# miczi/OpticalFlowHS

Hardware: AMD Instinct MI355X
Metric: Mpixel*iterations/sec (Horn-Schunck: derivative pass + Jacobi u/v sweeps, frames resident in HBM) (higher is better)
Workload: dtype f32; 1 GPU; a stream of 1920x1080 translating-texture pairs resident in HBM, a new pair every step (two seed pairs alternating), lambda 1, 100 Jacobi iterations, ITER|EPS (eps 1e-6) termination; width=1920, height=1080, iters=100, pairs_per_gpu=1, kernel=strip, fuse_steps=20, threads=1024, rows_per_lane_or_groups=5, tiles_per_launch=243, lds_bytes=131328, hipgraph=True, termination=ITER|EPS (eps 1e-6), loop=stream, call=hsflow_pipeline_submit_device, 6 slots on 2 streams, eps_rerun=0

## Files before the change

opticalflowhs_amd/csrc/hs_kernels_strip.hip.h:

```cpp
#pragma once
#include <type_traits>

#ifndef HS_SWEEP_STAMPS
#define HS_SWEEP_STAMPS 0
#endif
#ifndef HS_DIAG
#define HS_DIAG 0
#endif


namespace hsk {

struct StripGeom {
    int W, H, P;
    long long plane;
    int T, HX;
    int CW, CH;
    int NW;
    int tiles_x, tiles_y;
    int zero_in;
    int org;
    int ey0, ey1;
    const int *pair_list;
};

__device__ __forceinline__ int mirror_index(int i, int n)
{
    if (i < 0) i = -1 - i;
    if (i >= n) i = 2 * n - 1 - i;
    if ((unsigned)i >= (unsigned)n) {
        const int p = 2 * n;
        int m = i % p;
        if (m < 0) m += p;
        i = m < n ? m : p - 1 - m;
    }
    return i;
}

typedef float f2 __attribute__((ext_vector_type(2)));
typedef float f4 __attribute__((ext_vector_type(4)));

struct PersistArgs {
    unsigned *flags;
    unsigned *err;
    float *ub[2], *vb[2];
    int n_phase, T_last;
    unsigned wait_ticks;
};

typedef unsigned u4v __attribute__((ext_vector_type(4)));
__device__ __forceinline__ __amdgpu_buffer_rsrc_t plane_rsrc(float *p)
{
    return __builtin_amdgcn_make_buffer_rsrc((void *)p, 0, 0xFFFFFFFFu, 0x00020000);
}
__device__ __forceinline__ void store_f4_sc1(__amdgpu_buffer_rsrc_t rs, unsigned row_bytes, unsigned lane_bytes, f4 v)
{
    __builtin_amdgcn_raw_buffer_store_b128(__builtin_bit_cast(u4v, v), rs, (int)lane_bytes, (int)row_bytes, 16);
}
__device__ __forceinline__ f4 load_f4_sc1(__amdgpu_buffer_rsrc_t rs, unsigned row_bytes, unsigned lane_bytes)
{
    return __builtin_bit_cast(f4, __builtin_amdgcn_raw_buffer_load_b128(rs, (int)lane_bytes, (int)row_bytes, 16));
}
__device__ __forceinline__ unsigned load_u32_sc1(const unsigned *p)
{
    return __hip_atomic_load(p, __ATOMIC_RELAXED, __HIP_MEMORY_SCOPE_AGENT);
}

__device__ __forceinline__ int hs_lane_now()
{
    unsigned m = ~0u;
    asm volatile("" : "+s"(m));
    return (int)__builtin_amdgcn_mbcnt_hi(m, __builtin_amdgcn_mbcnt_lo(m, 0u));
}

__device__ __forceinline__ f2 f2_fma(f2 a, f2 b, f2 c) { return __builtin_elementwise_fma(a, b, c); }
__device__ __forceinline__ f2 f2_swap(f2 a) { return __builtin_shufflevector(a, a, 1, 0); }
__device__ __forceinline__ f2 sweep_diff(f2 o, f2 n) { return f2_fma(o, f2{4.0f, 4.0f}, -n); }
__device__ __forceinline__ float sweep_diff(float o, float n) { return fmaf(4.0f, o, -n); }

struct RowCoef { f2 alP, alQ, beP, beQ, gaP, gaQ; };

struct Cross { f2 uP, uQ, vP, vQ; };

__device__ __forceinline__ f2 pk_add_swapped(f2 a, f2 b)
{
    f2 r;
    asm("v_pk_add_f32 %0, %1, %2 op_sel:[0,1] op_sel_hi:[1,0]" : "=v"(r) : "v"(a), "v"(b));
    return r;
}

template <int E>
__device__ __forceinline__ void cross_rows(Cross &s, const f2 cuP, const f2 cuQ, const f2 cvP, const f2 cvQ,
                                           const f2 duP, const f2 duQ, const f2 dvP, const f2 dvQ)
{
    if (E == 0) {
        s.uP = duP + cuQ; s.uQ = duQ + cuP;
        s.vP = dvP + cvQ; s.vQ = dvQ + cvP;
    } else {
        s.uQ = pk_add_swapped(duQ, cuQ);
        s.uP.x = duP.x + wave_from_prev_lane(cuP.y); s.uP.y = duP.y + wave_from_next_lane(cuP.x);
        s.vQ = pk_add_swapped(dvQ, cvQ);
        s.vP.x = dvP.x + wave_from_prev_lane(cvP.y); s.vP.y = dvP.y + wave_from_next_lane(cvP.x);
    }
}

template <int E>
__device__ __forceinline__ void strip_row_update(f2 &uP, f2 &uQ, f2 &vP, f2 &vQ, const Cross &sc, const Cross &sp, RowCoef &c)
{
    f2 ubP, ubQ, vbP, vbQ;
    if (E == 0) {
        ubQ = pk_add_swapped(sc.uQ, sp.uQ);
        ubP.x = sc.uP.x + wave_from_prev_lane(sp.uP.y); ubP.y = sc.uP.y + wave_from_next_lane(sp.uP.x);
        vbQ = pk_add_swapped(sc.vQ, sp.vQ);
        vbP.x = sc.vP.x + wave_from_prev_lane(sp.vP.y); vbP.y = sc.vP.y + wave_from_next_lane(sp.vP.x);
    } else {
        ubP = sc.uP + sp.uQ; ubQ = sc.uQ + sp.uP;
        vbP = sc.vP + sp.vQ; vbQ = sc.vQ + sp.vP;
    }
    const f2 qP = f2_fma(c.alP, ubP, f2_fma(c.beP, vbP, c.gaP));
    const f2 qQ = f2_fma(c.alQ, ubQ, f2_fma(c.beQ, vbQ, c.gaQ));
    uP = f2_fma(-c.alP, qP, ubP);
    vP = f2_fma(-c.beP, qP, vbP);
    uQ = f2_fma(-c.alQ, qQ, ubQ);
    vQ = f2_fma(-c.beQ, qQ, vbQ);
    c.gaP *= 4.0f;
    c.gaQ *= 4.0f;
}

struct FrameSrc {
    int PA, PB;
    uint8_t *keepA, *keepB;
};

template <int R, bool EXT = false>
__device__ __forceinline__ void strip_derive(const uint8_t *__restrict__ fA, const uint8_t *__restrict__ fB,
                                             const StripGeom &g, long long base, int x0, int y0, int dir, bool xin,
                                             uint4 (&lc)[R], const FrameSrc fs = FrameSrc{0, 0, nullptr, nullptr},
                                             const unsigned keep = 0)
{
    const int PA = EXT ? fs.PA : g.P, PB = EXT ? fs.PB : g.P;
    const int mode = xin ? 0 : ((x0 < 0 || (g.W & 3) == 0) ? 1 : 2);
    int xg = x0, xb[4] = {0, 0, 0, 0};
    unsigned flipx = 0;
    if (mode == 1) {
        xg = x0 < 0 ? -x0 - 4 : 2 * g.W - x0 - 4;
        if (xg < 0 || xg + 4 > g.W) xg = 0;
        flipx = 0xFu;
    } else if (mode == 2) {
#pragma unroll
        for (int k = 0; k < 4; k++) {
            xb[k] = mirror_index(x0 + k, g.W);
            if (x0 + k >= g.W) flipx |= 1u << k;
        }
    }
    uint32_t wa[R + 2], wbv[R];
#pragma unroll
    for (int j = 0; j < R + 2; j++)
        wa[j] = *(const uint32_t *)(fA + base + (long long)mirror_index(y0 + dir * (j - 1), g.H) * PA + (mode == 2 ? 0 : xg));
#pragma unroll
    for (int r = 0; r < R; r++)
        wbv[r] = *(const uint32_t *)(fB + base + (long long)mirror_index(y0 + dir * r, g.H) * PB + (mode == 2 ? 0 : xg));
    if (mode == 1) {
#pragma unroll
        for (int j = 0; j < R + 2; j++) wa[j] = __builtin_bswap32(wa[j]);
#pragma unroll
        for (int r = 0; r < R; r++) wbv[r] = __builtin_bswap32(wbv[r]);
    }
    if (__builtin_amdgcn_ballot_w64(mode == 2) != 0) {
        if (mode == 2) {
            auto bytes = [&](const uint8_t *row) -> uint32_t {
                return (uint32_t)row[xb[0]] | ((uint32_t)row[xb[1]] << 8) | ((uint32_t)row[xb[2]] << 16) | ((uint32_t)row[xb[3]] << 24);
            };
#pragma unroll
            for (int j = 0; j < R + 2; j++) wa[j] = bytes(fA + base + (long long)mirror_index(y0 + dir * (j - 1), g.H) * PA);
#pragma unroll
            for (int r = 0; r < R; r++) wbv[r] = bytes(fB + base + (long long)mirror_index(y0 + dir * r, g.H) * PB);
        }
    }
    if constexpr (EXT) {
        if (fs.keepA != nullptr) {
#pragma unroll
            for (int r = 0; r < R; r++) {
                if ((keep >> r) & 1u) {
                    const long long o = base + (long long)(y0 + dir * r) * g.P + x0;
                    *(uint32_t *)(fs.keepA + o) = wa[r + 1];
                    *(uint32_t *)(fs.keepB + o) = wbv[r];
                }
            }
        }
    }
    int a[R + 2][6];
#pragma unroll
    for (int j = 0; j < R + 2; j++) {
        const uint32_t wd = wa[j];
        a[j][0] = (int)((uint32_t)__builtin_amdgcn_update_dpp(0, (int)wd, 0x138, 0xF, 0xF, true) >> 24);
        a[j][5] = (int)((uint32_t)__builtin_amdgcn_update_dpp(0, (int)wd, 0x130, 0xF, 0xF, true) & 0xFFu);
#pragma unroll
        for (int k = 0; k < 4; k++) a[j][k + 1] = (int)((wd >> (8 * k)) & 0xFFu);
    }
#pragma unroll
    for (int r = 0; r < R; r++) {
        const int y = y0 + dir * r;
        const uint32_t wb = wbv[r];
        const bool yflip = (y < 0 || y >= g.H) != (dir < 0);
        uint32_t o[4];
#pragma unroll
        for (int k = 0; k < 4; k++) {
            int ix8 = (a[r][k + 2] + 2 * a[r + 1][k + 2] + a[r + 2][k + 2]) - (a[r][k] + 2 * a[r + 1][k] + a[r + 2][k]);
            int iy8 = (a[r + 2][k] + 2 * a[r + 2][k + 1] + a[r + 2][k + 2]) - (a[r][k] + 2 * a[r][k + 1] + a[r][k + 2]);
            if ((flipx >> k) & 1u) ix8 = -ix8;
            if (yflip) iy8 = -iy8;
            o[k] = pack_deriv(ix8, iy8, (int)((wb >> (8 * k)) & 0xFFu) - a[r + 1][k + 1]);
        }
        lc[r] = make_uint4(o[0], o[1], o[2], o[3]);
    }
}


struct TileId { int tile, slot, pair, bx, by; };
template <bool LISTED, bool SCALAR>
__device__ __forceinline__ TileId tile_decode(const StripGeom &g)
{
    const int tpp = g.tiles_x * g.tiles_y;
    const int tile = xcd_contiguous_tile(blockIdx.x, gridDim.x);
    const int slot = tile / tpp;
    const int t2 = tile - slot * tpp;
    int pair = slot;
    if constexpr (LISTED) {
        if (g.pair_list) pair = g.pair_list[slot];
    }
    if constexpr (SCALAR) pair = __builtin_amdgcn_readfirstlane(pair);
    const int by = t2 / g.tiles_x, bx = t2 - by * g.tiles_x;
    return TileId{tile, slot, pair, bx, by};
}

#define HS_ROW_IN_CORE(j, y, T, CH, H) ((j) >= (T) && (j) < (T) + (CH) && (y) >= 0 && (y) < (H))
__device__ __forceinline__ bool row_in_core(const int j, const int y, const int T, const int CH, const int H)
{
    return HS_ROW_IN_CORE(j, y, T, CH, H);
}
__device__ __forceinline__ int row_dist(const int j, const int T, const int CH)
{
    return j < T ? T - j : (j >= T + CH ? j - (T + CH - 1) : 0);
}
__device__ __forceinline__ bool lane_in_core(const int x0, const int xl, const StripGeom &g)
{
    return (x0 >= 0) && (x0 < g.W) && (xl >= g.HX) && (xl < g.HX + g.CW);
}

__device__ __forceinline__ bool group_inside(const int x0, const int W) { return (x0 >= 0) && (x0 + 3 < W); }
struct ColRule { int xg, rev, slow; };
__device__ __forceinline__ ColRule column_rule(const int x0, const int W, const bool side, const bool inside)
{
    ColRule c{x0, 0, 0};
    if (side && !inside) {
        if (x0 < 0 && -x0 <= W) { c.xg = -x0 - 4; c.rev = 1; }
        else if (x0 >= W && (W & 3) == 0 && 2 * W - x0 - 4 >= 0) { c.xg = 2 * W - x0 - 4; c.rev = 1; }
        else { c.xg = 0; c.slow = 1; }
    }
    return c;
}

__device__ __forceinline__ void unpack(const float4 u, const float4 v, const uint4 cw, const float ilambda,
                                       f2 &uP, f2 &uQ, f2 &vP, f2 &vQ, RowCoef &c)
{
    constexpr int iPx = 0, iPy = 3, iQx = 1, iQy = 2;
    const float lu4[4] = {u.x, u.y, u.z, u.w}, lv4[4] = {v.x, v.y, v.z, v.w};
    uP = f2{lu4[iPx], lu4[iPy]}; uQ = f2{lu4[iQx], lu4[iQy]};
    vP = f2{lv4[iPx], lv4[iPy]}; vQ = f2{lv4[iQx], lv4[iQy]};
    float al[4], be[4], ga[4];
    const uint32_t cc[4] = {cw.x, cw.y, cw.z, cw.w};
#pragma unroll
    for (int p = 0; p < 4; p++) sweep_coefs(cc[p], ilambda, al[p], be[p], ga[p]);
    c.alP = f2{al[iPx], al[iPy]}; c.alQ = f2{al[iQx], al[iQy]};
    c.beP = f2{be[iPx], be[iPy]}; c.beQ = f2{be[iQx], be[iQy]};
    c.gaP = f2{ga[iPx], ga[iPy]} * 4.0f; c.gaQ = f2{ga[iQx], ga[iQy]} * 4.0f;
}

template <int R, bool DERIV, class RowOf>
__device__ __forceinline__ void load_rows(const uint32_t *coef, const float *u_in, const float *v_in, const StripGeom &g,
                                          const long long base, const int xg, const RowOf image_row,
                                          float4 (&lu)[R], float4 (&lv)[R], uint4 (&lc)[R])
{
#pragma unroll
    for (int r = 0; r < R; r++) {
        const long long off = base + (long long)mirror_index(image_row(r), g.H) * g.P + xg;
        const long long off_uv = g.zero_in ? (long long)xg : off;
        lc[r] = make_uint4(0u, 0u, 0u, 0u);
        if constexpr (!DERIV) {
            lu[r] = *(const float4 *)(u_in + off_uv);
            lv[r] = *(const float4 *)(v_in + off_uv);
            lc[r] = *(const uint4 *)(coef + off);
        } else {
            lu[r] = lv[r] = make_float4(0.f, 0.f, 0.f, 0.f);
        }
    }
    if constexpr (DERIV) {
        if (!g.zero_in) {
#pragma unroll
            for (int r = 0; r < R; r++) {
                const long long off = base + (long long)mirror_index(image_row(r), g.H) * g.P + xg;
                lu[r] = *(const float4 *)(u_in + off);
                lv[r] = *(const float4 *)(v_in + off);
            }
        }
    }
}

template <int R, bool DERIV, class RowOf>
__device__ __forceinline__ void load_rows_slow(const uint32_t *coef, const float *u_in, const float *v_in, const StripGeom &g,
                                               const float ilambda, const long long base, const int x0, const bool slow,
                                               const RowOf image_row, float4 (&lu)[R], float4 (&lv)[R], uint4 (&lc)[R],
                                               f2 (&uP)[R], f2 (&uQ)[R], f2 (&vP)[R], f2 (&vQ)[R], RowCoef (&cf)[R])
{
    if (__builtin_amdgcn_ballot_w64(slow) != 0) {
        if (slow) {
            const int xa = mirror_index(x0, g.W), xb = mirror_index(x0 + 1, g.W),
                      xc = mirror_index(x0 + 2, g.W), xd = mirror_index(x0 + 3, g.W);
#pragma unroll
            for (int r = 0; r < R; r++) {
                const long long row = base + (long long)mirror_index(image_row(r), g.H) * g.P;
                {
                    const float *uv = u_in + (g.zero_in ? 0 : row), *vv = v_in + (g.zero_in ? 0 : row);
                    lu[r] = make_float4(uv[xa], uv[xb], uv[xc], uv[xd]);
                    lv[r] = make_float4(vv[xa], vv[xb], vv[xc], vv[xd]);
                }
                if constexpr (!DERIV) {
                    const uint32_t *cv = coef + row;
                    lc[r] = make_uint4(cv[xa], cv[xb], cv[xc], cv[xd]);
                    unpack(lu[r], lv[r], lc[r], ilambda, uP[r], uQ[r], vP[r], vQ[r], cf[r]);
                }
            }
        }
    }
}

#define HS_MIRROR_ROW(DERIV, rev, lu, lv, uP, uQ, vP, vQ, cf)                                      \
    do {                                                                                           \
        if constexpr (DERIV) {                                                                     \
            if (rev) {                                                                             \
                lu = make_float4(lu.w, lu.z, lu.y, lu.x);                                          \
                lv = make_float4(lv.w, lv.z, lv.y, lv.x);                                          \
            }                                                                                      \
        } else {                                                                                   \
            uP = rev ? f2_swap(uP) : uP; uQ = rev ? f2_swap(uQ) : uQ;                              \
            vP = rev ? f2_swap(vP) : vP; vQ = rev ? f2_swap(vQ) : vQ;                              \
            cf.alP = rev ? f2_swap(cf.alP) : cf.alP; cf.alQ = rev ? f2_swap(cf.alQ) : cf.alQ;      \
            cf.beP = rev ? f2_swap(cf.beP) : cf.beP; cf.beQ = rev ? f2_swap(cf.beQ) : cf.beQ;      \
            cf.gaP = rev ? f2_swap(cf.gaP) : cf.gaP; cf.gaQ = rev ? f2_swap(cf.gaQ) : cf.gaQ;      \
        }                                                                                          \
    } while (0)

#define HS_LOAD_PHASE(R, DERIV, side, inside, x0, base, image_row, lu, lv, lc, uP, uQ, vP, vQ, cf)                     \
    do {                                                                                                               \
        const ColRule col_ = column_rule(x0, g.W, side, inside);                                                       \
        const bool mirrored_ = col_.rev != 0;                                                                          \
        load_rows<R, DERIV>(coef, u_in, v_in, g, base, col_.xg, image_row, lu, lv, lc);                                \
        if constexpr (!DERIV) {                                                                                        \
            _Pragma("unroll") for (int r = 0; r < R; r++)                                                              \
                unpack(lu[r], lv[r], lc[r], ilambda, uP[r], uQ[r], vP[r], vQ[r], cf[r]);                               \
        }                                                                                                              \
        if (side) {                                                                                                    \
            _Pragma("unroll") for (int r = 0; r < R; r++)                                                              \
                HS_MIRROR_ROW(DERIV, mirrored_, lu[r], lv[r], uP[r], uQ[r], vP[r], vQ[r], cf[r]);                      \
            load_rows_slow<R, DERIV>(coef, u_in, v_in, g, ilambda, base, x0, col_.slow != 0, image_row, lu, lv, lc,    \
                                     uP, uQ, vP, vQ, cf);                                                              \
        }                                                                                                              \
    } while (0)

template <int R, class RowOf>
__device__ __forceinline__ void store_deriv_rows(uint32_t *coef_w, const StripGeom &g, const long long base,
                                                 const int x0, const unsigned rowcore, const RowOf image_row, const uint4 (&lc)[R])
{
#pragma unroll
    for (int r = 0; r < R; r++)
        if ((rowcore >> r) & 1u) *(uint4 *)(coef_w + base + (long long)image_row(r) * g.P + x0) = lc[r];
}

template <int R, class RowOf>
__device__ __forceinline__ void store_flow_rows(float *u_out, float *v_out, const StripGeom &g,
                                                const long long base, const int x0, const unsigned rowcore, const RowOf image_row,
                                                const f2 (&uP)[R], const f2 (&uQ)[R], const f2 (&vP)[R], const f2 (&vQ)[R])
{
#pragma unroll
    for (int r = 0; r < R; r++) {
        if ((rowcore >> r) & 1u) {
            const long long off = base + (long long)image_row(r) * g.P + x0;
            const float fin = __builtin_ldexpf(1.0f, -2 * g.T);
            *(float4 *)(u_out + off) = make_float4(uP[r].x * fin, uQ[r].x * fin, uQ[r].y * fin, uP[r].y * fin);
            *(float4 *)(v_out + off) = make_float4(vP[r].x * fin, vQ[r].x * fin, vQ[r].y * fin, vP[r].y * fin);
        }
    }
}

__device__ __forceinline__ unsigned long long store_stamps(unsigned long long *stamps, const unsigned long long st0,
                                                           const unsigned long long sr0, const unsigned long long st1,
                                                           const unsigned long long st2, const int tile)
{
    __builtin_amdgcn_s_waitcnt(0);
    unsigned long long *o = stamps + (size_t)blockIdx.x * 8;
    o[0] = st0; o[1] = st1; o[2] = st2;
    const unsigned long long st3 = __builtin_amdgcn_s_memtime();
    o[3] = st3;
    o[4] = sr0; o[5] = __builtin_amdgcn_s_memrealtime();
    o[6] = (unsigned long long)__builtin_amdgcn_s_getreg(((4 - 1) << 11) | (0 << 6) | 20);
    o[7] = (unsigned long long)tile;
    return st3;
}

template <class Lane>
__device__ __forceinline__ void eps_put_max(const float *vals, const int NW, const Lane lane_id, unsigned *word)
{
    float x = lane_id() < NW ? vals[lane_id()] : 0.f;
    x = wave_max_nonneg(x);
    if (lane_id() == 0) *word = __float_as_uint(x);
}
#define HS_EPS_FOLD_SWEEP(EPS, e, s, w, NW, lane, eps_lds, eps_out, eps_stride)                                        \
    do {                                                                                                               \
        const float unscale_ = __builtin_ldexpf(1.0f, -2 * ((s) + 1));                                                 \
        if (EPS == 3) {                                                                                                \
            const float e_ = wave_max_nonneg(e) * unscale_;                                                            \
            if ((lane) == 0) eps_lds[16 + (w)] = e_;                                                                   \
        }                                                                                                              \
        if (EPS == 1) {                                                                                                \
            const float e_ = wave_max_nonneg(e) * unscale_;                                                            \
            if ((lane) == 0) eps_lds[((s) & 1) * 16 + (w)] = e_;                                                       \
            if ((s) > 0 && (w) == 0) {                                                                                 \
                float x_ = (lane) < (NW) ? eps_lds[(((s) - 1) & 1) * 16 + (lane)] : 0.f;                               \
                x_ = wave_max_nonneg(x_);                                                                              \
                if ((lane) == 0) eps_out[(size_t)((s) - 1) * (eps_stride) + blockIdx.x] = __float_as_uint(x_);         \
            }                                                                                                          \
        }                                                                                                              \
    } while (0)
template <int EPS, bool COUNTS, class Lane>
__device__ __forceinline__ void eps_tail(const int T, const int seen_n, const bool wit_sum, const int w, const int NW, const Lane lane_id,
                                         float *eps_lds, unsigned *eps_out, unsigned *wit_out, const int eps_stride)
{
    if (EPS == 1) {
        __syncthreads();
        if (w == 0) eps_put_max(eps_lds + ((T - 1) & 1) * 16, NW, lane_id, eps_out + (size_t)(T - 1) * eps_stride + blockIdx.x);
    }
    if (EPS == 2 || EPS == 3) {
        const int witnessed = EPS == 3 ? T - 1 : T;
        if (lane_id() == 0) eps_lds[w] = COUNTS ? (float)seen_n : (seen_n == witnessed ? __builtin_inff() : 0.f);
        __syncthreads();
        if (w == 0) {
            const float x = lane_id() < NW ? eps_lds[lane_id()] : 0.f;
            const float n = wit_sum ? wave_sum16(x) : wave_max_nonneg(x);
            if (lane_id() == 0) wit_out[blockIdx.x] = __float_as_uint(!COUNTS ? n : n == (float)witnessed ? __builtin_inff() : 0.f);
            if (EPS == 3) eps_put_max(eps_lds + 16, NW, lane_id, eps_out + (size_t)eps_stride + blockIdx.x);
        }
    }
}

constexpr int kSweepLast = 16;
template <int EPS, bool TWO, bool MARK_LAST = false, class Sweep>
__device__ __forceinline__ void run_sweeps(const int &T, const Sweep &sweep)
{
    constexpr int kLast = MARK_LAST ? kSweepLast : 0;
    if constexpr (EPS == 3) {
#pragma unroll 1
        for (int s = 0; s + 1 < T; s++) sweep(s, std::integral_constant<int, 2>{});
        sweep(T - 1, std::integral_constant<int, 1 + kLast>{});
    } else if constexpr (EPS != 1) {
        int s = 0;
        if constexpr (TWO) {
#pragma unroll 1
            for (; s + 2 < T; s += 2) {
                sweep(s, std::integral_constant<int, EPS>{});
                sweep(s + 1, std::integral_constant<int, EPS>{});
            }
        }
#pragma unroll 1
        for (; s + 1 < T; s++) sweep(s, std::integral_constant<int, EPS>{});
        sweep(T - 1, std::integral_constant<int, EPS + kLast>{});
    } else {
        const int n = T;
#pragma unroll 1
        for (int s = 0; s < n; s++) sweep(s, std::integral_constant<int, EPS>{});
    }
}

template <int R, int NTMAX, int EPS, int E0, bool DERIV, bool PERSIST = false>
__device__ __forceinline__ void strip_body(const uint32_t *__restrict__ coef,
                                                        const float *__restrict__ u_in,
                                                        const float *__restrict__ v_in,
                                                        float *__restrict__ u_out,
                                                        float *__restrict__ v_out, const StripGeom g,
                                                        const float ilambda,
                                                        unsigned *__restrict__ eps_out, const int eps_stride,
                                                        unsigned long long *__restrict__ stamps,
                                                        const float eps_thr, const uint8_t *__restrict__ fA,
                                                        const uint8_t *__restrict__ fB, uint32_t *__restrict__ coef_w,
                                                        const FrameSrc fs, const PersistArgs pa = PersistArgs())
{
    static_assert(!PERSIST || EPS == 0 || EPS == 2, "the persistent form runs plain or witness phases");
    extern __shared__ __attribute__((aligned(16))) float4 ex[];
    unsigned long long st0 = 0, sr0 = 0, st1 = 0, st2 = 0;
    if (stamps) { st0 = __builtin_amdgcn_s_memtime(); sr0 = __builtin_amdgcn_s_memrealtime(); }
    const int lane = threadIdx.x & 63;
    const int w = __builtin_amdgcn_readfirstlane(threadIdx.x >> 6);
    const int NW = g.NW;
    float *eps_lds = (float *)(ex + (size_t)2 * NW * 4 * 64);
    const TileId tl = tile_decode<!PERSIST, false>(g);
    const int x0 = tl.bx * g.CW - g.HX + 4 * lane;
    const int y0 = tl.by * g.CH - g.T + w * R;
    const long long base = (long long)tl.pair * g.plane;
    const bool xin = group_inside(x0, g.W);
    const bool rev = (R & 1) != 0 && ((y0 + g.org) & 1) != 0;
    auto img_row = [&](int r) { return rev ? R - 1 - r : r; };
    auto image_row = [&](int r) { return y0 + img_row(r); };

    f2 uP[R], uQ[R], vP[R], vQ[R];
    RowCoef cf[R];
    float4 lu[R], lv[R];
    uint4 lc[R];
    const int rx0 = tl.bx * g.CW - g.HX;
    const bool xedge = !(rx0 >= 0 && rx0 + 256 <= g.W);
    HS_LOAD_PHASE(R, DERIV, xedge, xin, x0, base, image_row, lu, lv, lc, uP, uQ, vP, vQ, cf);
    unsigned rowcore = 0;
    int rdist[R];
#pragma unroll
    for (int r = 0; r < R; r++) {
        const int j = w * R + img_row(r);
        const int y = image_row(r);
        if constexpr (DERIV) {
            if (row_in_core(j, y, g.T, g.CH, g.H)) rowcore |= 1u << r;
        } else {
            if (HS_ROW_IN_CORE(j, y, g.T, g.CH, g.H)) rowcore |= 1u << r;
        }
        rdist[r] = row_dist(j, g.T, g.CH);
    }
    const bool lanecore = lane_in_core(x0, 4 * lane, g);
    if constexpr (DERIV) {
        const unsigned keep = (fs.keepA != nullptr && lanecore) ? rowcore : 0u;
        strip_derive<R, true>(fA, fB, g, base, x0, rev ? y0 + R - 1 : y0, rev ? -1 : 1, xin, lc, fs, keep);
#pragma unroll
        for (int r = 0; r < R; r++) unpack(lu[r], lv[r], lc[r], ilambda, uP[r], uQ[r], vP[r], vQ[r], cf[r]);
    }
    const int pr = g.W - 1 - x0;
    constexpr bool LANE_HW = EPS != 0 || PERSIST;
    const auto lane_id = [&]() __attribute__((always_inline)) { return LANE_HW ? hs_lane_now() : lane; };
    unsigned epscore = 0;
    if (EPS != 0) {
#pragma unroll
        for (int r = 0; r < R; r++) {
            const int y = image_row(r);
            if (((rowcore >> r) & 1u) && y >= g.ey0 && y < g.ey1) epscore |= 1u << r;
        }
    }
    if (DERIV && lanecore) store_deriv_rows<R>(coef_w, g, base, x0, rowcore, image_row, lc);

#define HS_LIKELY(c) (PERSIST ? !!(c) : __builtin_expect(!!(c), 1))
#define HS_ACT(r) HS_LIKELY(((act >> (r)) & 1u) != 0u)
#define HS_ROW(r, PE, SC, SP)                                                                      \
    do {                                                                                           \
        if (HS_LIKELY(((actr >> (r)) & 1u) != 0u)) {                                               \
            f2 ouP, ouQ, ovP, ovQ;                                                                 \
            if (EM == 1) { ouP = uP[r]; ouQ = uQ[r]; ovP = vP[r]; ovQ = vQ[r]; }                   \
            if (HS_DIAG & 8) uP[r] += SC.uP + SP.uP;                                               \
            else strip_row_update<PE>(uP[r], uQ[r], vP[r], vQ[r], SC, SP, cf[r]);                  \
            if (EM == 1) {                                                                         \
                if ((epscore >> (r)) & 1u) {  \
                    const f2 dUP = sweep_diff(ouP, uP[r]), dUQ = sweep_diff(ouQ, uQ[r]), dVP = sweep_diff(ovP, vP[r]), dVQ = sweep_diff(ovQ, vQ[r]); \
                    if (HS_LIKELY(!xedge)) {  \
                        e = fmaxf(fmaxf(e, fabsf(dUP.x)), fabsf(dUP.y));                           \
                        e = fmaxf(fmaxf(e, fabsf(dUQ.x)), fabsf(dUQ.y));                           \
                        e = fmaxf(fmaxf(e, fabsf(dVP.x)), fabsf(dVP.y));                           \
                        e = fmaxf(fmaxf(e, fabsf(dVQ.x)), fabsf(dVQ.y));                           \
                    } else {                                                                       \
                         \
                        e = fmaxf(e, fmaxf(fabsf(dUP.x), fabsf(dVP.x)));                           \
                        if (pr >= 1) e = fmaxf(e, fmaxf(fabsf(dUQ.x), fabsf(dVQ.x)));              \
                        if (pr >= 2) e = fmaxf(e, fmaxf(fabsf(dUQ.y), fabsf(dVQ.y)));              \
                        if (pr >= 3) e = fmaxf(e, fmaxf(fabsf(dUP.y), fabsf(dVP.y)));              \
                    }                                                                              \
                }                                                                                  \
            }                                                                                      \
        }                                                                                          \
    } while (0)
#define HS_CROSS(S, PE, A, B)                                                                      \
    do {                                                                                           \
        if (HS_LIKELY(((actb >> (A)) & 1u) != 0u)) {                               \
            if (HS_DIAG & 8) S.uP = uP[A] + uP[B];                                                 \
            else cross_rows<PE>(S, uP[A], uQ[A], vP[A], vQ[A], uP[B], uQ[B], vP[B], vQ[B]);        \
        }                                                                                          \
    } while (0)
#define HS_PUBLISH(buf, ln)                                                                         \
    do {                                                                                           \
        float4 *exw = ex + ((size_t)((buf) * NW + w) * 4) * 64 + (ln);                             \
        exw[0] = make_float4(uP[0].x, uP[0].y, uQ[0].x, uQ[0].y);                                  \
        exw[64] = make_float4(vP[0].x, vP[0].y, vQ[0].x, vQ[0].y);                                 \
        exw[128] = make_float4(uP[R - 1].x, uP[R - 1].y, uQ[R - 1].x, uQ[R - 1].y);                \
        exw[192] = make_float4(vP[R - 1].x, vP[R - 1].y, vQ[R - 1].x, vQ[R - 1].y);                \
    } while (0)

    if (stamps) st1 = __builtin_amdgcn_s_memtime();
    const bool nrev = (R & 1) != 0 && !rev;
    const int wa = w > 0 ? w - 1 : w, sa = w > 0 ? (nrev ? 0 : 2) : 0;
    const int wb = w < NW - 1 ? w + 1 : w, sb = w < NW - 1 ? (nrev ? 2 : 0) : 2;
    const int wu = rev ? wb : wa, su = rev ? sb : sa;
    const int wd = rev ? wa : wb, sd = rev ? sa : sb;
    int seen_n = 0;
    const unsigned long long wit_mask = (epscore & 1u) ? __builtin_amdgcn_ballot_w64(lanecore) : 0ull;
    const int core_here = min(g.CH, g.H - tl.by * g.CH);
    const int wit_lo = (g.T + R - 1) / R, wit_n = (g.T + core_here) / R - wit_lo;
    const bool wit_rot = wit_n > 0;
    const int wit_per = wit_rot ? wit_n : 1;
    const int wit_cnt0 = !wit_rot ? 0 : (w >= wit_lo && w < wit_lo + wit_n) ? w - wit_lo : (1 << 30);
    int wit_cnt = wit_cnt0;
    int Tp = g.T;
    unsigned long long act_lo = 0, act_hi = 0;
    auto sweep = [&](const int s, auto em_tag) __attribute__((always_inline)) {
        constexpr int EM = decltype(em_tag)::value & (kSweepLast - 1);
        constexpr bool IN_LOOP = (decltype(em_tag)::value & kSweepLast) == 0;
#if HS_DIAG & 4
        unsigned act = ~0u;
#else
        unsigned act = (unsigned)((act_lo << s) >> 32) & (unsigned)(act_hi >> (24 + s));
#endif
        unsigned actb = act | (act >> 1), actr = act;
        if constexpr (EPS != 1) asm volatile("" : "+s"(act), "+s"(actb), "+s"(actr));
        const float thr_s = __int_as_float(__float_as_int(eps_thr) + ((s + 1) << 24));
#if HS_DIAG & 1
        const float4 hu4 = make_float4(uP[0].x, uP[0].y, uQ[0].x, uQ[0].y), hv4 = make_float4(vP[0].x, vP[0].y, vQ[0].x, vQ[0].y);
        const float4 du4 = make_float4(uP[R - 1].x, uP[R - 1].y, uQ[R - 1].x, uQ[R - 1].y), dv4 = make_float4(vP[R - 1].x, vP[R - 1].y, vQ[R - 1].x, vQ[R - 1].y);
#else
        const int lane_l = lane_id();
        const float4 *eu = ex + ((size_t)((s & 1) * NW + wu) * 4 + su) * 64 + lane_l;
        const float4 *ed = ex + ((size_t)((s & 1) * NW + wd) * 4 + sd) * 64 + lane_l;
        const float4 hu4 = eu[0], hv4 = eu[64];
        const float4 du4 = ed[0], dv4 = ed[64];
#endif
        const f2 huP = f2{hu4.x, hu4.y}, huQ = f2{hu4.z, hu4.w}, hvP = f2{hv4.x, hv4.y}, hvQ = f2{hv4.z, hv4.w};
        const f2 duP = f2{du4.x, du4.y}, duQ = f2{du4.z, du4.w}, dvP = f2{dv4.x, dv4.y}, dvQ = f2{dv4.z, dv4.w};

        float e = 0.f;
        constexpr int EL = E0 ^ ((R - 1) & 1);
        Cross sA, s0, sK, sL;
        const bool wturn = EM == 2 && (PERSIST ? wit_cnt == 0 : __builtin_expect(wit_cnt == 0, 0));
        float w0 = 0.f;
        if (wturn) w0 = uP[0].x;
        if (HS_ACT(0)) cross_rows<E0 ^ 1>(sA, huP, huQ, hvP, hvQ, uP[0], uQ[0], vP[0], vQ[0]);
        if (R == 1) {
            if (HS_ACT(0)) cross_rows<E0>(s0, uP[0], uQ[0], vP[0], vQ[0], duP, duQ, dvP, dvQ);
        } else {
            constexpr int R1 = R > 1 ? 1 : 0;
            HS_CROSS(s0, E0, 0, R1);
        }
        HS_ROW(0, E0, s0, sA);
        if (EM == 2) {
            if (wturn) seen_n += (__builtin_amdgcn_ballot_w64(fabsf(sweep_diff(w0, uP[0].x)) >= thr_s) & wit_mask) != 0 ? 1 : 0;
            wit_cnt = wturn ? wit_per - 1 : wit_cnt - 1;
        }
        if (R >= 2) {
            constexpr int RM = R > 2 ? R - 2 : 0;
            if (HS_ACT(R - 1)) cross_rows<EL>(sL, uP[R - 1], uQ[R - 1], vP[R - 1], vQ[R - 1], duP, duQ, dvP, dvQ);
                if (R >= 3) HS_CROSS(sK, EL ^ 1, RM, R - 1);
            if (R == 2) HS_ROW(R - 1, EL, sL, s0);
            else HS_ROW(R - 1, EL, sL, sK);
        }
#if !(HS_DIAG & 1)
        if (s + 1 < Tp) HS_PUBLISH((s + 1) & 1, lane_l);
#endif
        if (R >= 3) {
            Cross sp = s0;
            Cross scs[R], sc1;
#pragma unroll
            for (int r = 1; r < R - 1; r++) {
                Cross &sc = IN_LOOP && EM != 1 ? scs[r] : sc1;
                if (r == R - 2) sc = sK;
                else {
                    const int rn = r + 1 < R ? r + 1 : r;
                    if (r & 1) HS_CROSS(sc, E0 ^ 1, r, rn);
                    else HS_CROSS(sc, E0, r, rn);
                }
                if (r & 1) HS_ROW(r, E0 ^ 1, sc, sp);
                else HS_ROW(r, E0, sc, sp);
                sp = sc;
            }
        }
        if constexpr (EM == 1) HS_EPS_FOLD_SWEEP(EPS, lanecore ? e : 0.f, s, w, NW, lane_id(), eps_lds, eps_out, eps_stride);
#if !(HS_DIAG & 2)
        if (s + 1 < Tp) __syncthreads();
#endif
#if HS_SWEEP_STAMPS
        if (stamps && gridDim.x <= 8192 && threadIdx.x == 0)
            stamps[(size_t)gridDim.x * 8 + (size_t)blockIdx.x * 32 + (s & 31)] = __builtin_amdgcn_s_memtime();
#endif
    };
    if (rowcore == (1u << R) - 1u) __builtin_amdgcn_s_setprio(1);
    int ph = 0;
    unsigned flag_base = 0;
    unsigned long long pt_sweep = 0, pt_pub = 0, pt_wait = 0, pt_load = 0, pt0 = 0, pt_first = 0;
    if constexpr (PERSIST) {
        if (w == 0) flag_base = (unsigned)__builtin_amdgcn_readfirstlane((int)load_u32_sc1(pa.flags + tl.tile));
    }
#pragma unroll 1
    for (;;) {
    if constexpr (PERSIST) {
        Tp = ph == pa.n_phase - 1 ? pa.T_last : g.T;
        seen_n = 0;
        wit_cnt = wit_cnt0;
        if (stamps && ph == 0) pt_first = pt0 = __builtin_amdgcn_s_memtime();
    }
    {
        static_assert(R <= 8, "the trapezoid tables hold 8 rows per lane");
        const int n0 = min(max(g.T - Tp + 1 - w * R, -32), R), m0 = min(max(w * R + R + 1 - g.T - g.CH - Tp, -32), R);
        act_lo = ~0ull << (32 + (rev ? m0 : n0));
        act_hi = ~0ull >> (40 - R + (rev ? n0 : m0));
    }
    HS_PUBLISH(0, lane_id());
    __syncthreads();
    if (PERSIST && stamps && ph > 0) {
        const unsigned long long t = __builtin_amdgcn_s_memtime();
        pt_load += t - pt0;
        pt0 = t;
    }
    run_sweeps<EPS, false, true>(Tp, sweep);
    unsigned *const eps_ph = PERSIST ? eps_out + (size_t)ph * eps_stride : eps_out;
    eps_tail<EPS, true>(Tp, seen_n, wit_rot, w, NW, lane_id, eps_lds, eps_out, eps_ph, eps_stride);
    if (stamps) st2 = __builtin_amdgcn_s_memtime();

    if constexpr (!PERSIST) {
        int lane_s = lane_id();
        if constexpr (!LANE_HW) asm volatile("" : "+v"(lane_s));
        const int x0s = tl.bx * g.CW - g.HX + 4 * lane_s;
        if (lanecore) store_flow_rows<R>(u_out, v_out, g, base, x0s, rowcore, image_row, uP, uQ, vP, vQ);
        break;
    } else {
        if (stamps) { pt_sweep += st2 - pt0; pt0 = st2; }
        const __amdgpu_buffer_rsrc_t pu = plane_rsrc(pa.ub[ph & 1]), pv = plane_rsrc(pa.vb[ph & 1]);
        const float fin = __builtin_ldexpf(1.0f, -2 * Tp);
        const int lane_x = lane_id();
        const int x0x = tl.bx * g.CW - g.HX + 4 * lane_x;
        const ColRule colx = column_rule(x0x, g.W, xedge, group_inside(x0x, g.W));
        const int xgx = colx.xg;
        const bool xrevx = colx.rev != 0;
#pragma unroll
        for (int r = 0; r < R; r++) {
            if ((rowcore >> r) & 1u) {
                uP[r] *= fin; uQ[r] *= fin; vP[r] *= fin; vQ[r] *= fin;
                if (lanecore) {
                    const unsigned row = 4u * (unsigned)(base + (long long)image_row(r) * g.P);
                    store_f4_sc1(pu, row, 4u * (unsigned)x0x, f4{uP[r].x, uQ[r].x, uQ[r].y, uP[r].y});
                    store_f4_sc1(pv, row, 4u * (unsigned)x0x, f4{vP[r].x, vQ[r].x, vQ[r].y, vP[r].y});
                }
            }
        }
        if (ph == pa.n_phase - 1) break;
#pragma unroll
        for (int r = 0; r < R; r++) {
            const int nact = Tp - rdist[r] > 0 ? Tp - rdist[r] : 0;
            const float back = __builtin_ldexpf(1.0f, -2 * nact);
            cf[r].gaP *= back; cf[r].gaQ *= back;
        }
        asm volatile("s_waitcnt vmcnt(0)" ::: "memory");
        __syncthreads();
        if (stamps) { const unsigned long long t = __builtin_amdgcn_s_memtime(); pt_pub += t - pt0; pt0 = t; }
        int *const dead_lds = (int *)(eps_lds + 31);
        if (w == 0) {
            const unsigned target = flag_base + (unsigned)ph + 1u;
            if (lane_id() == 0) __hip_atomic_store(pa.flags + tl.tile, target, __ATOMIC_RELAXED, __HIP_MEMORY_SCOPE_AGENT);
            int nb = -1;
            if (lane_id() < 8) {
                const int k = lane_id() < 4 ? lane_id() : lane_id() + 1;
                const int nx = tl.bx + k % 3 - 1, ny = tl.by + k / 3 - 1;
                if (nx >= 0 && nx < g.tiles_x && ny >= 0 && ny < g.tiles_y) nb = tl.slot * g.tiles_x * g.tiles_y + ny * g.tiles_x + nx;
            } else if (lane_id() == 8) nb = (int)gridDim.x;
            const unsigned long long t0 = __builtin_amdgcn_s_memrealtime();
            int dead = 0;
            for (;;) {
                unsigned v = target;
                if (nb >= 0) v = load_u32_sc1(pa.flags + nb);
                const bool aborted = lane_id() == 8 && v != 0u;
                const bool behind = lane_id() < 8 && (int)(v - target) < 0;
                if (__builtin_amdgcn_ballot_w64(aborted) != 0) { dead = 1; break; }
                if (__builtin_amdgcn_ballot_w64(behind) == 0) break;
                if (__builtin_amdgcn_s_memrealtime() - t0 > (unsigned long long)pa.wait_ticks) {
                    dead = 1;
                    if (lane_id() == 0) {
                        __hip_atomic_store(pa.flags + gridDim.x, 1u, __ATOMIC_RELAXED, __HIP_MEMORY_SCOPE_AGENT);
                        __hip_atomic_store(pa.err, 1u, __ATOMIC_RELAXED, __HIP_MEMORY_SCOPE_SYSTEM);
                    }
                    break;
                }
                __builtin_amdgcn_s_sleep(4);
            }
            if (lane_id() == 0) *dead_lds = dead;
        }
        __syncthreads();
        if (__builtin_amdgcn_readfirstlane(*dead_lds)) return;
        if (stamps) { const unsigned long long t = __builtin_amdgcn_s_memtime(); pt_wait += t - pt0; pt0 = t; }
        {
            f4 tu[R], tv[R];
#pragma unroll
            for (int r = 0; r < R; r++) {
                const unsigned row = 4u * (unsigned)(base + (long long)mirror_index(image_row(r), g.H) * g.P);
                tu[r] = f4{uP[r].x, uQ[r].x, uQ[r].y, uP[r].y};
                tv[r] = f4{vP[r].x, vQ[r].x, vQ[r].y, vP[r].y};
                if (!((rowcore >> r) & 1u) || !lanecore) {
                    tu[r] = load_f4_sc1(pu, row, 4u * (unsigned)xgx);
                    tv[r] = load_f4_sc1(pv, row, 4u * (unsigned)xgx);
                }
            }
#pragma unroll
            for (int r = 0; r < R; r++) {
                if (xrevx) {
                    tu[r] = f4{tu[r].w, tu[r].z, tu[r].y, tu[r].x};
                    tv[r] = f4{tv[r].w, tv[r].z, tv[r].y, tv[r].x};
                }
                uP[r] = f2{tu[r].x, tu[r].w}; uQ[r] = f2{tu[r].y, tu[r].z};
                vP[r] = f2{tv[r].x, tv[r].w}; vQ[r] = f2{tv[r].y, tv[r].z};
            }
        }
        ph++;
    }
    }
#undef HS_ROW
#undef HS_ACT
#undef HS_LIKELY
#undef HS_CROSS
#undef HS_PUBLISH
    if (stamps && threadIdx.x == 0) {
        const unsigned long long st3 = store_stamps(stamps, st0, sr0, st1, st2, tl.tile);
        if (PERSIST && gridDim.x <= 8192) {
            unsigned long long *q = stamps + (size_t)gridDim.x * 8 + (size_t)blockIdx.x * 32;
            q[0] = pt_sweep; q[1] = pt_pub; q[2] = pt_wait; q[3] = pt_load; q[4] = pt_first - st1; q[5] = st3 - st2;
        }
    }
}

template <int R, int NTMAX, int EPS, int E0>
__global__ __launch_bounds__(NTMAX) void k_jacobi_strip(const uint32_t *__restrict__ coef,
                                                        const float *__restrict__ u_in,
                                                        const float *__restrict__ v_in,
                                                        float *__restrict__ u_out,
                                                        float *__restrict__ v_out, const StripGeom g,
                                                        const float ilambda,
                                                        unsigned *__restrict__ eps_out, const int eps_stride,
                                                        unsigned long long *__restrict__ stamps,
                                                        const float eps_thr)
{
    strip_body<R, NTMAX, EPS, E0, false>(coef, u_in, v_in, u_out, v_out, g, ilambda, eps_out, eps_stride, stamps, eps_thr,
                                     nullptr, nullptr, nullptr, FrameSrc{0, 0, nullptr, nullptr});
}

template <int R, int NTMAX, int EPS, int E0>
__global__ __launch_bounds__(NTMAX) void k_jacobi_strip_deriv(const uint8_t *__restrict__ fA,
                                                              const uint8_t *__restrict__ fB, const FrameSrc fs,
                                                              uint32_t *__restrict__ coef_w,
                                                              const float *__restrict__ u_in,
                                                              const float *__restrict__ v_in,
                                                              float *__restrict__ u_out,
                                                              float *__restrict__ v_out, const StripGeom g,
                                                              const float ilambda,
                                                              unsigned *__restrict__ eps_out, const int eps_stride,
                                                              unsigned long long *__restrict__ stamps,
                                                              const float eps_thr)
{
    strip_body<R, NTMAX, EPS, E0, true>(nullptr, u_in, v_in, u_out, v_out, g, ilambda, eps_out, eps_stride, stamps, eps_thr,
                                    fA, fB, coef_w, fs);
}

template <int R, int NTMAX, int EPS, int E0, bool DERIV>
__global__ __launch_bounds__(NTMAX) void k_jacobi_strip_persist(const uint8_t *__restrict__ fA,
                                                                const uint8_t *__restrict__ fB,
                                                                uint32_t *coef_rw,
                                                                const float *__restrict__ u_in,
                                                                const float *__restrict__ v_in, const StripGeom g,
                                                                const float ilambda,
                                                                unsigned *__restrict__ eps_out, const int eps_stride,
                                                                unsigned long long *__restrict__ stamps,
                                                                const float eps_thr, const PersistArgs pa)
{
    strip_body<R, NTMAX, EPS, E0, DERIV, true>(coef_rw, u_in, v_in, nullptr, nullptr, g, ilambda, eps_out, eps_stride, stamps, eps_thr,
                                               fA, fB, coef_rw, FrameSrc{g.P, g.P, nullptr, nullptr}, pa);
}

__device__ __forceinline__ float lane_xor32(float x, bool lower)
{
    const unsigned b = __float_as_uint(x);
    const auto r = __builtin_amdgcn_permlane32_swap(b, b, false, false);
    return __uint_as_float(lower ? r[0] : r[1]);
}

template <int R, int NTMAX, int EPS, int E0, bool DERIV>
__device__ __forceinline__ void fold_body(const uint32_t *__restrict__ coef,
                                                       const float *__restrict__ u_in,
                                                       const float *__restrict__ v_in,
                                                       float *__restrict__ u_out,
                                                       float *__restrict__ v_out, const StripGeom g,
                                                       const float ilambda,
                                                       unsigned *__restrict__ eps_out, const int eps_stride,
                                                       unsigned long long *__restrict__ stamps,
                                                       const float eps_thr, const uint8_t *__restrict__ fA,
                                                       const uint8_t *__restrict__ fB, uint32_t *__restrict__ coef_w)
{
    extern __shared__ __attribute__((aligned(16))) float4 ex[];
    unsigned long long st0 = 0, sr0 = 0, st1 = 0, st2 = 0;
    if (stamps) { st0 = __builtin_amdgcn_s_memtime(); sr0 = __builtin_amdgcn_s_memrealtime(); }
    const int lane = threadIdx.x & 63, hl = lane & 31;
    const bool lower = lane >= 32;
    const int w = __builtin_amdgcn_readfirstlane(threadIdx.x >> 6);
    const int NW = g.NW;
    float *eps_lds = (float *)(ex + (size_t)2 * NW * 2 * 2 * 32);
    const TileId tl = tile_decode<true, true>(g);
    const int rx0 = tl.bx * g.CW - g.HX;
    const int x0 = rx0 + 4 * hl;
    const int yb = tl.by * g.CH - g.T + w * 2 * R;
    const long long base = (long long)tl.pair * g.plane;
    const bool xin = group_inside(x0, g.W);
    auto blk_row = [&](int r) { return lower ? 2 * R - 1 - r : r; };
    auto image_row = [&](int r) { return yb + blk_row(r); };
    const auto lane_id = [&]() { return lane; };

    f2 uP[R], uQ[R], vP[R], vQ[R];
    RowCoef cf[R];
    float4 lu[R], lv[R];
    uint4 lc[R];
    const bool side = !(rx0 >= 0 && rx0 + 128 <= g.W);
    HS_LOAD_PHASE(R, DERIV, side, xin, x0, base, image_row, lu, lv, lc, uP, uQ, vP, vQ, cf);
    if constexpr (DERIV) {
        strip_derive<R>(fA, fB, g, base, x0, lower ? yb + 2 * R - 1 : yb, lower ? -1 : 1, xin, lc);
#pragma unroll
        for (int r = 0; r < R; r++) unpack(lu[r], lv[r], lc[r], ilambda, uP[r], uQ[r], vP[r], vQ[r], cf[r]);
    }
    unsigned rowcore = 0;
    int rdist[R];
#pragma unroll
    for (int r = 0; r < R; r++) {
        const int jl = w * 2 * R + blk_row(r), y = image_row(r);
        if (HS_ROW_IN_CORE(jl, y, g.T, g.CH, g.H)) rowcore |= 1u << r;
        const int du = row_dist(w * 2 * R + r, g.T, g.CH), dd = row_dist(w * 2 * R + 2 * R - 1 - r, g.T, g.CH);
        rdist[r] = du < dd ? du : dd;
    }
    const bool lanecore = lane_in_core(x0, 4 * hl, g);
    const int pr = g.W - 1 - x0;
    if (DERIV && lanecore) store_deriv_rows<R>(coef_w, g, base, x0, rowcore, image_row, lc);

#define HF_ROW(r, PE, SC, SP)                                                                      \
    do {                                                                                           \
        if (rdist[r] <= last) {                                                                    \
            f2 ouP, ouQ, ovP, ovQ;                                                                 \
            if (EM == 1) { ouP = uP[r]; ouQ = uQ[r]; ovP = vP[r]; ovQ = vQ[r]; }                   \
            strip_row_update<PE>(uP[r], uQ[r], vP[r], vQ[r], SC, SP, cf[r]);                       \
            if (EM == 1) {                                                                         \
                if (((rowcore >> (r)) & 1u) && lanecore) {                                         \
                       \
                    e = fmaxf(e, fmaxf(fabsf(sweep_diff(ouP.x, uP[r].x)), fabsf(sweep_diff(ovP.x, vP[r].x))));           \
                    if (pr >= 1) e = fmaxf(e, fmaxf(fabsf(sweep_diff(ouQ.x, uQ[r].x)), fabsf(sweep_diff(ovQ.x, vQ[r].x)))); \
                    if (pr >= 2) e = fmaxf(e, fmaxf(fabsf(sweep_diff(ouQ.y, uQ[r].y)), fabsf(sweep_diff(ovQ.y, vQ[r].y)))); \
                    if (pr >= 3) e = fmaxf(e, fmaxf(fabsf(sweep_diff(ouP.y, uP[r].y)), fabsf(sweep_diff(ovP.y, vP[r].y)))); \
                }                                                                                  \
            }                                                                                      \
        }                                                                                          \
        __builtin_amdgcn_sched_barrier(0);                                                         \
    } while (0)
#define HF_CROSS(S, PE, A, B)                                                                      \
    do {                                                                                           \
        if (rdist[A] <= last || rdist[B] <= last)                                                  \
            cross_rows<PE>(S, uP[A], uQ[A], vP[A], vQ[A], uP[B], uQ[B], vP[B], vQ[B]);             \
    } while (0)
#define HF_SLOT(buf, ww, hh) (ex + ((size_t)(((buf) * NW + (ww)) * 2 + (hh)) * 2) * 32)
#define HF_PUBLISH(buf)                                                                            \
    do {                                                                                           \
        float4 *exw = HF_SLOT(buf, w, lower ? 1 : 0) + hl;                                         \
        exw[0] = make_float4(uP[0].x, uP[0].y, uQ[0].x, uQ[0].y);                                  \
        exw[32] = make_float4(vP[0].x, vP[0].y, vQ[0].x, vQ[0].y);                                 \
    } while (0)

    HF_PUBLISH(0);
    __syncthreads();
    if (stamps) st1 = __builtin_amdgcn_s_memtime();
    const int wo = lower ? (w < NW - 1 ? w + 1 : w) : (w > 0 ? w - 1 : w);
    const int ho = lower ? (w < NW - 1 ? 0 : 1) : (w > 0 ? 1 : 0);
    int seen_n = 0;
    const unsigned long long wit_mask = __builtin_amdgcn_ballot_w64((rowcore & 1u) && lanecore);
    auto sweep = [&](const int s, auto em_tag) __attribute__((always_inline)) {
        constexpr int EM = decltype(em_tag)::value;
        const int last = g.T - 1 - s;
        const float thr_s = __int_as_float(__float_as_int(eps_thr) + ((s + 1) << 24));
        const float4 *eo = HF_SLOT(s & 1, wo, ho) + hl;
        const float4 h4u = eo[0], h4v = eo[32];
        const f2 ouP_ = f2{h4u.x, h4u.y}, ouQ_ = f2{h4u.z, h4u.w}, ovP_ = f2{h4v.x, h4v.y}, ovQ_ = f2{h4v.z, h4v.w};
        const f2 iuP = f2{lane_xor32(uP[R - 1].x, lower), lane_xor32(uP[R - 1].y, lower)};
        const f2 iuQ = f2{lane_xor32(uQ[R - 1].x, lower), lane_xor32(uQ[R - 1].y, lower)};
        const f2 ivP = f2{lane_xor32(vP[R - 1].x, lower), lane_xor32(vP[R - 1].y, lower)};
        const f2 ivQ = f2{lane_xor32(vQ[R - 1].x, lower), lane_xor32(vQ[R - 1].y, lower)};
        float e = 0.f;
        const float w0 = uP[0].x;
        Cross sp, sc;
        if (rdist[0] <= last) cross_rows<E0 ^ 1>(sp, ouP_, ouQ_, ovP_, ovQ_, uP[0], uQ[0], vP[0], vQ[0]);
#pragma unroll
        for (int r = 0; r < R; r++) {
            const int rn = r + 1 < R ? r + 1 : r;
            if (r == R - 1) {
                if (rdist[r] <= last) {
                    if (r & 1) cross_rows<E0 ^ 1>(sc, uP[r], uQ[r], vP[r], vQ[r], iuP, iuQ, ivP, ivQ);
                    else cross_rows<E0>(sc, uP[r], uQ[r], vP[r], vQ[r], iuP, iuQ, ivP, ivQ);
                }
            } else if (r & 1) HF_CROSS(sc, E0 ^ 1, r, rn);
            else HF_CROSS(sc, E0, r, rn);
            if (r & 1) HF_ROW(r, E0 ^ 1, sc, sp);
            else HF_ROW(r, E0, sc, sp);
            if (r == 0) {
                if (EM == 2)
                    seen_n += (__builtin_amdgcn_ballot_w64(fabsf(sweep_diff(w0, uP[0].x)) >= thr_s) & wit_mask) != 0 ? 1 : 0;
                if (s + 1 < g.T) HF_PUBLISH((s + 1) & 1);
            }
            sp = sc;
        }
        if constexpr (EM == 1) HS_EPS_FOLD_SWEEP(EPS, e, s, w, NW, lane, eps_lds, eps_out, eps_stride);
        if (s + 1 < g.T) __syncthreads();
    };
    run_sweeps<EPS, true>(g.T, sweep);
    eps_tail<EPS, false>(g.T, seen_n, false, w, NW, lane_id, eps_lds, eps_out, eps_out, eps_stride);
#undef HF_ROW
#undef HF_CROSS
#undef HF_PUBLISH
#undef HF_SLOT
    if (stamps) st2 = __builtin_amdgcn_s_memtime();

    if (lanecore) store_flow_rows<R>(u_out, v_out, g, base, x0, rowcore, image_row, uP, uQ, vP, vQ);
    if (stamps && threadIdx.x == 0) store_stamps(stamps, st0, sr0, st1, st2, tl.tile);
}

template <int R, int NTMAX, int EPS, int E0>
__global__ __launch_bounds__(NTMAX) void k_jacobi_fold(const uint32_t *__restrict__ coef,
                                                       const float *__restrict__ u_in,
                                                       const float *__restrict__ v_in,
                                                       float *__restrict__ u_out,
                                                       float *__restrict__ v_out, const StripGeom g,
                                                       const float ilambda,
                                                       unsigned *__restrict__ eps_out, const int eps_stride,
                                                       unsigned long long *__restrict__ stamps,
                                                       const float eps_thr)
{
    fold_body<R, NTMAX, EPS, E0, false>(coef, u_in, v_in, u_out, v_out, g, ilambda, eps_out, eps_stride, stamps, eps_thr,
                                    nullptr, nullptr, nullptr);
}

template <int R, int NTMAX, int EPS, int E0>
__global__ __launch_bounds__(NTMAX) void k_jacobi_fold_deriv(const uint8_t *__restrict__ fA,
                                                             const uint8_t *__restrict__ fB,
                                                             uint32_t *__restrict__ coef_w,
                                                             const float *__restrict__ u_in,
                                                             const float *__restrict__ v_in,
                                                             float *__restrict__ u_out,
                                                             float *__restrict__ v_out, const StripGeom g,
                                                             const float ilambda,
                                                             unsigned *__restrict__ eps_out, const int eps_stride,
                                                             unsigned long long *__restrict__ stamps,
                                                             const float eps_thr)
{
    fold_body<R, NTMAX, EPS, E0, true>(nullptr, u_in, v_in, u_out, v_out, g, ilambda, eps_out, eps_stride, stamps, eps_thr,
                                   fA, fB, coef_w);
}

#undef HS_ROW_IN_CORE
#undef HS_EPS_FOLD_SWEEP
#undef HS_LOAD_PHASE
#undef HS_MIRROR_ROW

}
```

Baseline: 1.802 million Mpix*iter/s.

## Add unguarded full-strip sweep variant with scheduling barriers for interior waves

```diff
diff --git a/opticalflowhs_amd/csrc/hs_kernels_strip.hip.h b/opticalflowhs_amd/csrc/hs_kernels_strip.hip.h
--- a/opticalflowhs_amd/csrc/hs_kernels_strip.hip.h
+++ b/opticalflowhs_amd/csrc/hs_kernels_strip.hip.h
@@ -454,30 +454,31 @@
 }
 
 constexpr int kSweepLast = 16;
-template <int EPS, bool TWO, bool MARK_LAST = false, class Sweep>
+constexpr int kSweepFull = 32;
+template <int EPS, bool TWO, bool MARK_LAST = false, int MORE = 0, class Sweep>
 __device__ __forceinline__ void run_sweeps(const int &T, const Sweep &sweep)
 {
     constexpr int kLast = MARK_LAST ? kSweepLast : 0;
     if constexpr (EPS == 3) {
 #pragma unroll 1
-        for (int s = 0; s + 1 < T; s++) sweep(s, std::integral_constant<int, 2>{});
+        for (int s = 0; s + 1 < T; s++) sweep(s, std::integral_constant<int, 2 + MORE>{});
         sweep(T - 1, std::integral_constant<int, 1 + kLast>{});
     } else if constexpr (EPS != 1) {
         int s = 0;
         if constexpr (TWO) {
 #pragma unroll 1
             for (; s + 2 < T; s += 2) {
-                sweep(s, std::integral_constant<int, EPS>{});
-                sweep(s + 1, std::integral_constant<int, EPS>{});
+                sweep(s, std::integral_constant<int, EPS + MORE>{});
+                sweep(s + 1, std::integral_constant<int, EPS + MORE>{});
             }
         }
 #pragma unroll 1
-        for (; s + 1 < T; s++) sweep(s, std::integral_constant<int, EPS>{});
+        for (; s + 1 < T; s++) sweep(s, std::integral_constant<int, EPS + MORE>{});
         sweep(T - 1, std::integral_constant<int, EPS + kLast>{});
     } else {
         const int n = T;
 #pragma unroll 1
-        for (int s = 0; s < n; s++) sweep(s, std::integral_constant<int, EPS>{});
+        for (int s = 0; s < n; s++) sweep(s, std::integral_constant<int, EPS + MORE>{});
     }
 }
 
@@ -552,10 +553,15 @@
     if (DERIV && lanecore) store_deriv_rows<R>(coef_w, g, base, x0, rowcore, image_row, lc);
 
 #define HS_LIKELY(c) (PERSIST ? !!(c) : __builtin_expect(!!(c), 1))
-#define HS_ACT(r) HS_LIKELY(((act >> (r)) & 1u) != 0u)
+#define HS_GUARD(c) (FULL || HS_LIKELY(c))
+#define HS_FENCE()                                                                                 \
+    do {                                                                                           \
+        if constexpr (FULL) __builtin_amdgcn_sched_barrier(0);                                     \
+    } while (0)
+#define HS_ACT(r) HS_GUARD(((act >> (r)) & 1u) != 0u)
 #define HS_ROW(r, PE, SC, SP)                                                                      \
     do {                                                                                           \
-        if (HS_LIKELY(((actr >> (r)) & 1u) != 0u)) {                                               \
+        if (HS_GUARD(((actr >> (r)) & 1u) != 0u)) {                                                \
             f2 ouP, ouQ, ovP, ovQ;                                                                 \
             if (EM == 1) { ouP = uP[r]; ouQ = uQ[r]; ovP = vP[r]; ovQ = vQ[r]; }                   \
             if (HS_DIAG & 8) uP[r] += SC.uP + SP.uP;                                               \
@@ -578,13 +584,15 @@
                 }                                                                                  \
             }                                                                                      \
         }                                                                                          \
+        HS_FENCE();                                                                                \
     } while (0)
 #define HS_CROSS(S, PE, A, B)                                                                      \
     do {                                                                                           \
-        if (HS_LIKELY(((actb >> (A)) & 1u) != 0u)) {                               \
+        if (HS_GUARD(((actb >> (A)) & 1u) != 0u)) {                                \
             if (HS_DIAG & 8) S.uP = uP[A] + uP[B];                                                 \
             else cross_rows<PE>(S, uP[A], uQ[A], vP[A], vQ[A], uP[B], uQ[B], vP[B], vQ[B]);        \
         }                                                                                          \
+        if constexpr (!DERIV) HS_FENCE();                                                          \
     } while (0)
 #define HS_PUBLISH(buf, ln)                                                                         \
     do {                                                                                           \
@@ -614,19 +622,19 @@
     auto sweep = [&](const int s, auto em_tag) __attribute__((always_inline)) {
         constexpr int EM = decltype(em_tag)::value & (kSweepLast - 1);
         constexpr bool IN_LOOP = (decltype(em_tag)::value & kSweepLast) == 0;
-#if HS_DIAG & 4
+        constexpr bool FULL = (decltype(em_tag)::value & kSweepFull) != 0;
         unsigned act = ~0u;
-#else
-        unsigned act = (unsigned)((act_lo << s) >> 32) & (unsigned)(act_hi >> (24 + s));
+#if !(HS_DIAG & 4)
+        if constexpr (!FULL) act = (unsigned)((act_lo << s) >> 32) & (unsigned)(act_hi >> (24 + s));
 #endif
         unsigned actb = act | (act >> 1), actr = act;
-        if constexpr (EPS != 1) asm volatile("" : "+s"(act), "+s"(actb), "+s"(actr));
+        if constexpr (EPS != 1 && !FULL) asm volatile("" : "+s"(act), "+s"(actb), "+s"(actr));
         const float thr_s = __int_as_float(__float_as_int(eps_thr) + ((s + 1) << 24));
 #if HS_DIAG & 1
         const float4 hu4 = make_float4(uP[0].x, uP[0].y, uQ[0].x, uQ[0].y), hv4 = make_float4(vP[0].x, vP[0].y, vQ[0].x, vQ[0].y);
         const float4 du4 = make_float4(uP[R - 1].x, uP[R - 1].y, uQ[R - 1].x, uQ[R - 1].y), dv4 = make_float4(vP[R - 1].x, vP[R - 1].y, vQ[R - 1].x, vQ[R - 1].y);
 #else
-        const int lane_l = lane_id();
+        const int lane_l = FULL ? hs_lane_now() : lane_id();
         const float4 *eu = ex + ((size_t)((s & 1) * NW + wu) * 4 + su) * 64 + lane_l;
         const float4 *ed = ex + ((size_t)((s & 1) * NW + wd) * 4 + sd) * 64 + lane_l;
         const float4 hu4 = eu[0], hv4 = eu[64];
@@ -640,8 +648,12 @@
         Cross sA, s0, sK, sL;
         const bool wturn = EM == 2 && (PERSIST ? wit_cnt == 0 : __builtin_expect(wit_cnt == 0, 0));
         float w0 = 0.f;
-        if (wturn) w0 = uP[0].x;
+        if (wturn) {
+            w0 = uP[0].x;
+            if constexpr (FULL) asm volatile("" : "+v"(w0));
+        }
         if (HS_ACT(0)) cross_rows<E0 ^ 1>(sA, huP, huQ, hvP, hvQ, uP[0], uQ[0], vP[0], vQ[0]);
+        if constexpr (!DERIV) HS_FENCE();
         if (R == 1) {
             if (HS_ACT(0)) cross_rows<E0>(s0, uP[0], uQ[0], vP[0], vQ[0], duP, duQ, dvP, dvQ);
         } else {
@@ -656,6 +668,7 @@
         if (R >= 2) {
             constexpr int RM = R > 2 ? R - 2 : 0;
             if (HS_ACT(R - 1)) cross_rows<EL>(sL, uP[R - 1], uQ[R - 1], vP[R - 1], vQ[R - 1], duP, duQ, dvP, dvQ);
+            if constexpr (!DERIV) HS_FENCE();
                 if (R >= 3) HS_CROSS(sK, EL ^ 1, RM, R - 1);
             if (R == 2) HS_ROW(R - 1, EL, sL, s0);
             else HS_ROW(R - 1, EL, sL, sK);
@@ -663,6 +676,7 @@
 #if !(HS_DIAG & 1)
         if (s + 1 < Tp) HS_PUBLISH((s + 1) & 1, lane_l);
 #endif
+        HS_FENCE();
         if (R >= 3) {
             Cross sp = s0;
             Cross scs[R], sc1;
@@ -689,7 +703,8 @@
             stamps[(size_t)gridDim.x * 8 + (size_t)blockIdx.x * 32 + (s & 31)] = __builtin_amdgcn_s_memtime();
 #endif
     };
-    if (rowcore == (1u << R) - 1u) __builtin_amdgcn_s_setprio(1);
+    const bool full_strip = rowcore == (1u << R) - 1u;
+    if (full_strip) __builtin_amdgcn_s_setprio(1);
     int ph = 0;
     unsigned flag_base = 0;
     unsigned long long pt_sweep = 0, pt_pub = 0, pt_wait = 0, pt_load = 0, pt0 = 0, pt_first = 0;
@@ -717,7 +732,14 @@
         pt_load += t - pt0;
         pt0 = t;
     }
-    run_sweeps<EPS, false, true>(Tp, sweep);
+    if constexpr (!PERSIST && (EPS == 0 || EPS == 2) && R >= 4) {
+        unsigned take_full = (unsigned)__builtin_amdgcn_readfirstlane(full_strip ? 1 : 0), take_guarded;
+        asm volatile("" : "+s"(take_full));
+        if (take_full != 0u) run_sweeps<EPS, false, true, kSweepFull>(Tp, sweep);
+        take_guarded = take_full ^ 1u;
+        asm volatile("" : "+s"(take_guarded));
+        if (take_guarded != 0u) run_sweeps<EPS, false, true>(Tp, sweep);
+    } else run_sweeps<EPS, false, true>(Tp, sweep);
     unsigned *const eps_ph = PERSIST ? eps_out + (size_t)ph * eps_stride : eps_out;
     eps_tail<EPS, true>(Tp, seen_n, wit_rot, w, NW, lane_id, eps_lds, eps_out, eps_ph, eps_stride);
     if (stamps) st2 = __builtin_amdgcn_s_memtime();
@@ -820,6 +842,8 @@
 #undef HS_ROW
 #undef HS_ACT
 #undef HS_LIKELY
+#undef HS_GUARD
+#undef HS_FENCE
 #undef HS_CROSS
 #undef HS_PUBLISH
     if (stamps && threadIdx.x == 0) {
```

Result: no change. 1.789 million Mpix*iter/s (-0.7%).
